# labhamlet/wavjepa

Measured on AMD Instinct MI355X. Metric: jepa_pretrain_clips_per_sec, higher is better.
Workload: dtype bf16

## Files before the change

### include/wavjepa_hip.h

```cpp
#ifndef WAVJEPA_HIP_H
#define WAVJEPA_HIP_H
#include <stdint.h>

#ifdef __cplusplus
extern "C" {
#endif

#define WJ_ABI_VERSION 16
int wj_abi_version(void);
int wj_device_count(void);
int wj_struct_size(const char* name);

enum {
    WJ_EPI_BF16 = 0,
    WJ_EPI_BIAS_GELU2 = 1,
    WJ_EPI_MUL_GELU_GRAD = 2,
    WJ_EPI_ADD_F32 = 3,
    WJ_EPI_ATOMIC_F32 = 4,
    WJ_EPI_CONV_GELU = 5,
    WJ_EPI_BIAS_GELU = 6,
    WJ_EPI_BF16_ADD_POS = 8,
    WJ_EPI_MUL_GELU_GRAD_Z = 7
};
typedef struct {
    const void* A;
    const void* B;
    void* C;
    void* C2;
    const void* bias;
    const void* aux;
    float* colsum;
    const int32_t* rowmap;
    int64_t lda, ldb, ldc;
    int32_t M, N, K;
    int32_t a_trans, b_trans;
    int32_t epilogue;
    int32_t split_k;
    int32_t seg_rows, seg_valid;
    float alpha;
    void* workspace;
    int64_t workspace_bytes;
    int32_t schedule;
    int32_t persist_cus;
} wj_gemm_args;
int wj_gemm_bf16(const wj_gemm_args*, void* stream);
int wj_gemm_release_stream(void* stream);
typedef struct {
    const void* A;
    const void* B;
    const void* scale_a;
    const void* scale_b;
    void* C;
    void* C2;
    const float* bias;
    void* q_out;
    void* q_scales;
    int64_t lda, ldb, ldc;
    int64_t ld_scale_a, ld_scale_b, ld_q_scale;
    int32_t M, N, K;
    int32_t epilogue;
} wj_gemm_fp8_args;
int wj_gemm_mxfp8(const wj_gemm_fp8_args*, void* stream);

typedef struct {
    const void* x;
    void* q;
    void* scales;
    int64_t ldx, ldq, ld_scale;
    int32_t M, K;
} wj_quantize_fp8_args;
int wj_quantize_mxfp8(const wj_quantize_fp8_args*, void* stream);

typedef struct {
    const void* A[8];
    const void* B[8];
    void* C[8];
    int64_t lda[8], ldb[8], ldc[8];
    int32_t M[8], N[8], K[8];
    int32_t n;
} wj_wgrad_group_args;
int wj_wgrad_grouped(const wj_wgrad_group_args*, void* stream);

// ... 379 lines not shown
```

### wavjepa_amd/csrc/gemm_panel.hip

```cpp
#include <atomic>
#include "common.h"
#include "../../include/wavjepa_hip.h"
#include "gemm_internal.h"

namespace {

constexpr int NT = 512;
constexpr int PN = 384;
constexpr int THIRDS = PN / 128;
constexpr unsigned SLOT = 16384u;
constexpr unsigned A_RING = 0u, B_RING = 4u * SLOT;
constexpr unsigned BIAS_OFF = 8u * SLOT;
constexpr unsigned STRIP_OFF = BIAS_OFF + 2048u;
constexpr unsigned STRIP_ROW = 144u;
constexpr int LDS_TOTAL = (int)(STRIP_OFF + 8u * 16u * STRIP_ROW);
constexpr int EPI_STORES = 4 * THIRDS;

typedef __attribute__((ext_vector_type(4))) unsigned u32x4;
typedef __attribute__((ext_vector_type(2))) unsigned u32x2;

struct QArgs {
    const char* A;
    const char* B;
    char* C;
    const float* bias;
    long ldc_b;
    unsigned lda_b, ldb_b;
    int M, K, nitems, wpx;
    int diag;
};

template <int N>
__device__ __forceinline__ void wait_vmcnt() {
    asm volatile("s_waitcnt vmcnt(%0)" ::"n"(N) : "memory");
}

__device__ __forceinline__ void dma(unsigned voff, const char* sbase, unsigned lds_dst) {
    asm volatile("s_mov_b32 m0, %2\n\ts_nop 0\n\tglobal_load_lds_dwordx4 %0, %1" ::"v"(voff), "s"(sbase), "s"(lds_dst) : "memory", "m0");
}

__device__ __forceinline__ unsigned pack_bf16(float a, float b) {
    bf16x2 p;
    p[0] = f2bf(a);
    p[1] = f2bf(b);
    return __builtin_bit_cast(unsigned, p);
}

struct Cursor {
    int b_kt, b_sub;
    int a_it, a_kt;
};

template <int SUB, int PB, int PA>
__device__ __forceinline__ void step(f32x4 (&acc)[4][2 * THIRDS], bf16x8 (&af)[2][4][2], bf16x8 (&bf)[2][2][2], char* smem, const QArgs& a,
                                     Cursor& cur, unsigned& slot_b, unsigned& slot_a, int nk, int n_my, int q0, int cstart,
                                     const unsigned (&voff)[4], const unsigned (&dpiece)[4], unsigned a_rd, unsigned b_rd, bool a_wave,
                                     int& lag_w, int& lag_a, int rot) {
    __builtin_amdgcn_sched_barrier(0);
    if (!a_wave) {
        if (lag_w > 0) { wait_vmcnt<8 + EPI_STORES>(); --lag_w; }
        else wait_vmcnt<8>();
    } else if constexpr (SUB == THIRDS - 1) {
        if (lag_a > 0) { wait_vmcnt<12 + EPI_STORES>(); --lag_a; }
        else wait_vmcnt<12>();
    }
    asm volatile("s_waitcnt lgkmcnt(0)" ::: "memory");
    __builtin_amdgcn_s_barrier();
    __builtin_amdgcn_sched_barrier(0);
    {
        const int bk = cur.b_kt + rot < nk ? cur.b_kt + rot : cur.b_kt + rot - nk;
        const char* sb = a.B + (long)(cur.b_sub * 128) * a.ldb_b + (long)bk * 128;
        const unsigned dst = B_RING + slot_b * SLOT;
        if (!a_wave) {
            const char* src = (WJ_LAB_BUILD && (a.diag & 1)) ? a.B : sb;
            const unsigned mask = (WJ_LAB_BUILD && (a.diag & 1)) ? 0u : ~0u;
#pragma unroll
            for (int u = 0; u < 4; ++u) dma(voff[u] & mask, src, dpiece[u] + dst);
        }
        slot_b = (slot_b + 1) & 3;
        if (++cur.b_sub == THIRDS) { cur.b_sub = 0; if (++cur.b_kt == nk) cur.b_kt = 0; }
    }
    if constexpr (SUB == 0) {
        const int it = cur.a_it < n_my ? cur.a_it : n_my - 1;
        const int m0 = min((cstart + q0 + it * a.wpx) * 128, a.M - 128);
        const int ak = cur.a_kt + rot < nk ? cur.a_kt + rot : cur.a_kt + rot - nk;
        const char* sa = a.A + (long)m0 * a.lda_b + (long)ak * 128;
        const unsigned dst = A_RING + slot_a * SLOT;
        if (a_wave) {
            const char* src = (WJ_LAB_BUILD && (a.diag & 2)) ? a.A : sa;
            const unsigned mask = (WJ_LAB_BUILD && (a.diag & 2)) ? 0u : ~0u;
#pragma unroll
            for (int u = 0; u < 4; ++u) dma(voff[u] & mask, src, dpiece[u] + dst);
        }
        slot_a = (slot_a + 1) & 3;
        if (++cur.a_kt == nk) { cur.a_kt = 0; ++cur.a_it; }
    }
// ... 28 lines not shown
    __builtin_amdgcn_sched_barrier(0);
}

__device__ __forceinline__ void epilogue(f32x4 (&acc)[4][2 * THIRDS], char* smem, const QArgs& a, int m0, int wave, int lane) {
    const int wm = wave >> 2, wn = wave & 3;
    const int i = lane & 15, g = lane >> 4;
    char* strip = smem + STRIP_OFF + wave * (16 * STRIP_ROW);
    char* wr = strip + i * STRIP_ROW + g * 8;
    const int srow = lane >> 2, schunk = lane & 3;
    const char* rd = strip + srow * STRIP_ROW + schunk * 16;
    char* c0 = a.C + (long)(m0 + wm * 64 + srow) * a.ldc_b + (long)(wn * 32) * 2 + schunk * 16;
    const float* bias = reinterpret_cast<const float*>(smem + BIAS_OFF) + wn * 32 + 4 * g;
#pragma unroll
    for (int t = 0; t < THIRDS; ++t) {
        f32x4 bv[2];
#pragma unroll
        for (int ni = 0; ni < 2; ++ni) bv[ni] = *reinterpret_cast<const f32x4*>(bias + t * 128 + ni * 16);
#pragma unroll
        for (int mi = 0; mi < 4; ++mi) {
#pragma unroll
            for (int ni = 0; ni < 2; ++ni) {
                const f32x4 v = acc[mi][t * 2 + ni] + bv[ni];
                *reinterpret_cast<u32x2*>(wr + ni * 32) = u32x2{pack_bf16(v[0], v[1]), pack_bf16(v[2], v[3])};
            }
            __builtin_amdgcn_wave_barrier();
            const u32x4 o = *reinterpret_cast<const u32x4*>(rd);
            __builtin_amdgcn_wave_barrier();
            char* dst = (WJ_LAB_BUILD && (a.diag & 16)) ? a.C + (lane & 7) * 16 : c0 + (long)(mi * 16) * a.ldc_b + (long)(t * 128) * 2;
            __builtin_nontemporal_store(o, reinterpret_cast<u32x4*>(dst));
        }
    }
}

__global__ __launch_bounds__(NT, 1) void gemm_panel_kernel(QArgs a) {
    extern __shared__ __attribute__((aligned(16))) char smem[];
    const int t = threadIdx.x, lane = t & 63;
    const int wave = __builtin_amdgcn_readfirstlane(t >> 6);
    const int wm = wave >> 2, wn = wave & 3;
    const bool a_wave = wave < 4;
    const int nk = a.K >> 6;
    const unsigned lds0 = (unsigned)(size_t)(__attribute__((address_space(3))) char*)smem;

    const int xl = blockIdx.x & 7, q0 = blockIdx.x >> 3;
    const int qn = a.nitems >> 3, qr = a.nitems & 7;
    const int clen = qn + (xl < qr ? 1 : 0);
    const int cstart = xl < qr ? xl * (qn + 1) : qr * (qn + 1) + (xl - qr) * qn;
    if (q0 >= clen) return;
    const int n_my = (clen - q0 + a.wpx - 1) / a.wpx;

    if (t < PN) reinterpret_cast<float*>(smem + BIAS_OFF)[t] = a.bias ? a.bias[t] : 0.f;

    unsigned dpiece[4], voff[4];
    const unsigned ld_b = a_wave ? a.lda_b : a.ldb_b;
#pragma unroll
    for (int u = 0; u < 4; ++u) {
        const int r0 = 32 * (wave & 3) + 8 * u;
        dpiece[u] = lds0 + (unsigned)r0 * 128u;
        const int row = r0 + (lane >> 3);
        voff[u] = (unsigned)row * ld_b + (unsigned)(((lane & 7) ^ ((row >> 1) & 7)) * 16);
    }
    const int i = lane & 15, g = lane >> 4;
    const unsigned sw = (unsigned)((g ^ ((i >> 1) & 7)) << 4);
    const unsigned a_rd = (unsigned)((wm * 64 + i) * 128) + sw;
    const unsigned b_rd = (unsigned)((wn * 32 + i) * 128) + sw;

    const int rot = (WJ_LAB_BUILD && (a.diag & 32)) ? (q0 + 3 * xl) % nk : 0;
    auto phys = [&](int kt) { return kt + rot < nk ? kt + rot : kt + rot - nk; };
    Cursor cur;
    cur.a_it = 0; cur.a_kt = 4; cur.b_kt = 1; cur.b_sub = 1;
    if (cur.a_kt == nk) { cur.a_kt = 0; cur.a_it = 1; }
    {
        const int m0 = min((cstart + q0) * 128, a.M - 128);
#pragma unroll
        for (int k = 0; k < 4; ++k) {
            if (a_wave) {
                const char* sa = a.A + (long)m0 * a.lda_b + (long)phys(k) * 128;
#pragma unroll
                for (int u = 0; u < 4; ++u) dma(voff[u], sa, dpiece[u] + A_RING + k * SLOT);
            } else {
                const int kt = k / THIRDS, sub = k - kt * THIRDS;
                const char* sb = a.B + (long)(sub * 128) * a.ldb_b + (long)phys(kt) * 128;
#pragma unroll
                for (int u = 0; u < 4; ++u) dma(voff[u], sb, dpiece[u] + B_RING + k * SLOT);
            }
        }
    }
    f32x4 acc[4][2 * THIRDS];
    bf16x8 af[2][4][2], bf[2][2][2];
    wait_vmcnt<12>();
    asm volatile("s_waitcnt lgkmcnt(0)" ::: "memory");
    __builtin_amdgcn_s_barrier();
    __builtin_amdgcn_sched_barrier(0);
#pragma unroll
    for (int ni = 0; ni < 2; ++ni) {
        bf[0][ni][0] = *reinterpret_cast<const bf16x8*>(smem + B_RING + b_rd + ni * 2048);
        bf[0][ni][1] = *reinterpret_cast<const bf16x8*>(smem + B_RING + (b_rd ^ 64u) + ni * 2048);
    }
#pragma unroll
    for (int mi = 0; mi < 4; ++mi) {
        af[0][mi][0] = *reinterpret_cast<const bf16x8*>(smem + A_RING + a_rd + mi * 2048);
        af[0][mi][1] = *reinterpret_cast<const bf16x8*>(smem + A_RING + (a_rd ^ 64u) + mi * 2048);
    }
    unsigned slot_b = 0, slot_a = 0;
    int lag_w = 0, lag_a = 0;

    for (int it = 0; it < n_my; ++it) {
        const int m0 = min((cstart + q0 + it * a.wpx) * 128, a.M - 128);
#pragma unroll
        for (int mi = 0; mi < 4; ++mi)
#pragma unroll
            for (int c = 0; c < 2 * THIRDS; ++c) acc[mi][c] = f32x4{0.f, 0.f, 0.f, 0.f};
        for (int kt = 0; kt < nk; kt += 2) {
            step<0, 0, 0>(acc, af, bf, smem, a, cur, slot_b, slot_a, nk, n_my, q0, cstart, voff, dpiece, a_rd, b_rd, a_wave, lag_w, lag_a, rot);
            step<1, 1, 0>(acc, af, bf, smem, a, cur, slot_b, slot_a, nk, n_my, q0, cstart, voff, dpiece, a_rd, b_rd, a_wave, lag_w, lag_a, rot);
            step<2, 0, 0>(acc, af, bf, smem, a, cur, slot_b, slot_a, nk, n_my, q0, cstart, voff, dpiece, a_rd, b_rd, a_wave, lag_w, lag_a, rot);
            step<0, 1, 1>(acc, af, bf, smem, a, cur, slot_b, slot_a, nk, n_my, q0, cstart, voff, dpiece, a_rd, b_rd, a_wave, lag_w, lag_a, rot);
            step<1, 0, 1>(acc, af, bf, smem, a, cur, slot_b, slot_a, nk, n_my, q0, cstart, voff, dpiece, a_rd, b_rd, a_wave, lag_w, lag_a, rot);
            step<2, 1, 1>(acc, af, bf, smem, a, cur, slot_b, slot_a, nk, n_my, q0, cstart, voff, dpiece, a_rd, b_rd, a_wave, lag_w, lag_a, rot);
        }
        __builtin_amdgcn_sched_barrier(0);
        asm volatile("s_nop 7\n\ts_nop 7" ::: "memory");
        epilogue(acc, smem, a, m0, wave, lane);
        __builtin_amdgcn_sched_barrier(0);
        lag_w = 3;
        lag_a = 3;
    }
    wait_vmcnt<0>();
    __builtin_amdgcn_s_barrier();
}


}

bool wj_gemm_panel_eligible(const wj_gemm_args* a) {
    if (a->a_trans || a->b_trans || a->rowmap || a->split_k > 1 || a->colsum || a->aux) return false;
    if (a->epilogue != WJ_EPI_BF16) return false;
    if (a->N != PN || a->M < 128) return false;
    if (a->K < 256 || (a->K % 128)) return false;
    if ((a->lda & 7) || (a->ldb & 7) || (a->ldc & 7)) return false;
    if (((uintptr_t)a->A | (uintptr_t)a->B | (uintptr_t)a->C | (uintptr_t)a->bias) & 15) return false;
    if (a->lda * 2 * 128 >= (1l << 31) || a->ldb * 2 * 128 >= (1l << 31)) return false;
    return true;
}

int wj_gemm_panel_launch(const wj_gemm_args* a, hipStream_t s) {
    if (!wj_gemm_panel_eligible(a)) return WJ_ERR_UNSUPPORTED;
    QArgs p;
    p.A = (const char*)a->A; p.B = (const char*)a->B; p.C = (char*)a->C; p.bias = (const float*)a->bias;
    p.ldc_b = a->ldc * 2; p.lda_b = (unsigned)(a->lda * 2); p.ldb_b = (unsigned)(a->ldb * 2);
    p.M = a->M; p.K = a->K;
    p.nitems = (a->M + 127) / 128;
    p.wpx = a->persist_cus > 0 ? (a->persist_cus > 32 ? 32 : a->persist_cus) : 32;
    p.diag = wj_lab_env_int("WJ_PANEL_DIAG", 0);
    int dev = 0;
    if (hipGetDevice(&dev) != hipSuccess || dev < 0 || dev >= 32) return WJ_ERR_UNSUPPORTED;
    static std::atomic<bool> lds_ok[32];
    if (!lds_ok[dev].load(std::memory_order_acquire)) {
        if (hipFuncSetAttribute((const void*)gemm_panel_kernel, hipFuncAttributeMaxDynamicSharedMemorySize, LDS_TOTAL) != hipSuccess) return WJ_ERR_LAUNCH;
        lds_ok[dev].store(true, std::memory_order_release);
    }
    hipLaunchKernelGGL(gemm_panel_kernel, dim3(8 * p.wpx), dim3(NT), LDS_TOTAL, s, p);
    WJ_CHECK_LAUNCH();
    return WJ_OK;
}
```

### wavjepa_amd/csrc/misc.hip

```cpp
#include <string.h>
#include "common.h"
#include "../../include/wavjepa_hip.h"
#ifdef WJ_LAB
#include "../../include/wavjepa_hip_lab.h"
#endif

namespace {

inline int grid_for(long n_items, int per_block, int cap = 8192) {
    long g = (n_items + per_block - 1) / per_block;
    if (g < 1) g = 1;
    return (int)(g > cap ? cap : g);
}

__global__ __launch_bounds__(256) void gelu_bwd_kernel(const bf16_t* __restrict__ dpost, const bf16_t* __restrict__ pre,
                                                       bf16_t* __restrict__ dpre, long n8) {
    for (long i = blockIdx.x * 256L + threadIdx.x; i < n8; i += (long)gridDim.x * 256) {
        const bf16x8 d = *reinterpret_cast<const bf16x8*>(dpost + i * 8);
        const bf16x8 p = *reinterpret_cast<const bf16x8*>(pre + i * 8);
        bf16x8 o;
#pragma unroll
        for (int e = 0; e < 8; ++e) o[e] = f2bf(bf2f(d[e]) * gelu_grad_f(bf2f(p[e])));
        *reinterpret_cast<bf16x8*>(dpre + i * 8) = o;
    }
// ... 506 lines not shown
        const int c = (int)(i / a.length), l = (int)(i - (long)c * a.length);
        const float d = src[(long)c * a.L_full + start + l] - mean;
        q += d * d;
    }
    const float stdv = sqrtf(block_sum(q, red) / (float)(n - 1));
    const float inv = 1.0f / (stdv + 1e-5f);
    const int orow = a.perm_inv ? a.perm_inv[bs] : bs;
    bf16_t* out = (bf16_t*)a.out + (long)orow * n;
    for (long i = threadIdx.x; i < n; i += 1024) {
        const int c = (int)(i / a.length), l = (int)(i - (long)c * a.length);
        out[i] = f2bf((src[(long)c * a.L_full + start + l] - mean) * inv);
    }
}

}

#define STREAM ((hipStream_t)stream)

extern "C" int wj_abi_version(void) { return WJ_ABI_VERSION; }
extern "C" int wj_device_count(void) {
    int n = 0;
    if (hipGetDeviceCount(&n) != hipSuccess) return 0;
    return n;
}

extern "C" int wj_struct_size(const char* name) {
    if (!name) return -1;
#define WJ_SZ(T) if (!strcmp(name, #T)) return (int)sizeof(T);
    WJ_SZ(wj_gemm_args) WJ_SZ(wj_ln_fwd_args) WJ_SZ(wj_ln_bwd_args) WJ_SZ(wj_colsum_args) WJ_SZ(wj_attn_fwd_args)
    WJ_SZ(wj_attn_bwd_args) WJ_SZ(wj_conv0_fwd_args) WJ_SZ(wj_conv0_bwd_args) WJ_SZ(wj_gelu_bwd_args) WJ_SZ(wj_conv_w_args)
    WJ_SZ(wj_add_pos_args) WJ_SZ(wj_gather_args) WJ_SZ(wj_scatter_fill_args) WJ_SZ(wj_scatter_fill_bwd_args)
    WJ_SZ(wj_unmask_rows_args) WJ_SZ(wj_instnorm_args) WJ_SZ(wj_mse_args) WJ_SZ(wj_ema_args) WJ_SZ(wj_sumsq_args)
    WJ_SZ(wj_adamw_args) WJ_SZ(wj_cast_args) WJ_SZ(wj_crop_args) WJ_SZ(wj_zero_rows_args) WJ_SZ(wj_instnorm_mean_args) WJ_SZ(wj_spin_args)
    WJ_SZ(wj_gemm_fp8_args) WJ_SZ(wj_quantize_fp8_args) WJ_SZ(wj_wgrad_group_args) WJ_SZ(wj_rir_conv_args) WJ_SZ(wj_snr_mix_args) WJ_SZ(wj_resample_args) WJ_SZ(wj_mse_groups_args) WJ_SZ(wj_transpose_args) WJ_SZ(wj_colsum_group_args) WJ_SZ(wj_rccl_init_args) WJ_SZ(wj_rccl_launch_args) WJ_SZ(wj_rccl_wait_args)
#ifdef WJ_LAB
    WJ_SZ(wj_collective_footprint_args)
#endif
#undef WJ_SZ
    return -1;
}

int64_t wj_gemm_ws_bytes(const wj_gemm_args* a);
int64_t wj_conv0_fwd_ws_bytes(const wj_conv0_fwd_args* a);
int64_t wj_conv0_bwd_ws_bytes(const wj_conv0_bwd_args* a);
int64_t wj_rir_conv_ws_bytes(const wj_rir_conv_args* a);
int64_t wj_snr_mix_ws_bytes(const wj_snr_mix_args* a);
int64_t wj_mse_groups_ws_bytes(const wj_mse_groups_args* a);

extern "C" int64_t wj_workspace_bytes(const char* fn, const void* args) {
    if (!fn || !args) return -1;
    if (!strcmp(fn, "wj_gemm_bf16")) return wj_gemm_ws_bytes((const wj_gemm_args*)args);
    if (!strcmp(fn, "wj_mask_scatter_fill_pos_bwd")) {
        const wj_scatter_fill_bwd_args* a = (const wj_scatter_fill_bwd_args*)args;
        return (int64_t)wj_scatter_fill_bwd_partial_rows(a->B, a->T) * a->D * 4;
    }
    if (!strcmp(fn, "wj_layernorm_bwd")) return 1536LL * 3 * ((const wj_ln_bwd_args*)args)->D * 4;
    if (!strcmp(fn, "wj_attn_bwd")) {
        const wj_attn_bwd_args* a = (const wj_attn_bwd_args*)args;
        return (int64_t)a->B * 3 * a->H * a->hd * 4;
    }
    if (!strcmp(fn, "wj_conv0_gn_gelu_fwd")) return wj_conv0_fwd_ws_bytes((const wj_conv0_fwd_args*)args);
    if (!strcmp(fn, "wj_conv0_gn_gelu_bwd")) return wj_conv0_bwd_ws_bytes((const wj_conv0_bwd_args*)args);
    if (!strcmp(fn, "wj_masked_mse")) {
        const wj_mse_args* a = (const wj_mse_args*)args;
        return (2 + (int64_t)a->B * a->G * a->T) * 4;
    }
    if (!strcmp(fn, "wj_grad_sumsq")) return 1024 * 4;
// ... 257 lines not shown
```

### wavjepa_amd/engine.py

```python
from __future__ import annotations

from dataclasses import dataclass
from typing import Dict, List, Optional, Sequence, Tuple

import numpy as np
import torch

from . import ops
from .params import FlatParams


def _empty(*shape, dtype, device):
    import os
    if os.environ.get("WJ_ARENA_FILL", "") == "nan":
        if not dtype.is_floating_point:
            return torch.full(shape, 0x7f, dtype=dtype, device=device)
        return torch.full(shape, float("nan"), dtype=dtype, device=device)
    return torch.empty(*shape, dtype=dtype, device=device)


@dataclass
class EngineConfig:
    conv_spec: Sequence[Tuple[int, int, int]]
    in_channels: int
# ... 249 lines not shown
        self.stacks = list(cfg.conv_prefixes)
        assert len(self.stacks) in (1, self.S)
        self.C = cfg.conv_spec[-1][0]
        assert all(c == self.C for c, _, _ in cfg.conv_spec), "all conv layers must have the same width"
        assert cfg.d_enc % cfg.h_enc == 0 and cfg.d_dec % cfg.h_dec == 0
        self.N = 0
        self.G = 0
        import os as _os
        self.use_side = _os.environ.get("WJ_SIDE_STREAM", "1") != "0"
        self._opt_ev = None
        self.ragged = _os.environ.get("WJ_RAGGED", "1") != "0"
        self.ragged_step = False
        self.sparse_conv = _os.environ.get("WJ_SPARSE_CONV", "1") != "0" and all(k >= st for _, k, st in cfg.conv_spec[1:])
        self._conv_grads_dirty = False
        self.fuse_conv_gelu_bwd = _os.environ.get("WJ_FUSE_CONV_GELU_BWD", "1") != "0"
        self.trim_tail = _os.environ.get("WJ_TRIM_TAIL", "1") != "0"
        self.tail = None
        self.fp8 = _os.environ.get("WJ_FP8", "0") == "1"
        self._w8: Dict[int, Tuple[torch.Tensor, torch.Tensor, int, int]] = {}
        self._a8: Dict[str, Tuple[torch.Tensor, torch.Tensor]] = {}
        self.side = self._pick_side_stream() if self.use_side else torch.cuda.Stream(device=self.dev)
        self.has_mapper = "post_extraction_mapper.weight" in flat.by_name
        self.wt_dgrad = _os.environ.get("WJ_WT_DGRAD", "1") != "0"
        self.pair_split = _os.environ.get("WJ_PAIR_SPLIT", "0") == "1"
        self.pair_ws = None
        self._conv_w_fresh = False
        self.defer_folds = _os.environ.get("WJ_DEFER_FOLDS", "1") != "0"
        self.fuse_add_pos = _os.environ.get("WJ_FUSE_ADD_POS", "1") != "0"
        self.mapper_wgrad_side = _os.environ.get("WJ_MAPPER_WGRAD_SIDE", "1") != "0"
        self.conv_wgrad_side = _os.environ.get("WJ_CONV_WGRAD_SIDE", "1") != "0"
        lean = _os.environ.get("WJ_LN_LEAN", "")
        self.ln_lean = {t.strip() for t in lean.replace("+", ",").split(",") if t.strip() and t.strip() != "0"} if self.use_side else set()
        self.ln_lean_wgs = int(_os.environ.get("WJ_LN_LEAN_WGS", "256"))
        self._lean_now = False
        self._folds = []
        self._bind_params()
        self._bind_wt()
        self._conv_w: Dict[str, torch.Tensor] = {}
        self._alloc_conv_weights()

    def _pick_side_stream(self) -> torch.cuda.Stream:
        main = torch.cuda.current_stream(self.dev)
        ticks = 20000
        ops.spin(100, stream=main.cuda_stream)

        def pair_ms(cand: torch.cuda.Stream) -> float:
            e0, e1, go, done = (torch.cuda.Event(enable_timing=True) for _ in range(4))
            best = 1e9
            for _ in range(2):
                go.record(main)
                cand.wait_event(go)
                e0.record(main)
                ops.spin(ticks, stream=main.cuda_stream)
                ops.spin(ticks, stream=cand.cuda_stream)
                done.record(cand)
                main.wait_event(done)
                e1.record(main)
                e1.synchronize()
                best = min(best, e0.elapsed_time(e1))
            return best

        def single_ms() -> float:
            e0, e1 = torch.cuda.Event(enable_timing=True), torch.cuda.Event(enable_timing=True)
            e0.record(main)
            ops.spin(ticks, stream=main.cuda_stream)
            e1.record(main)
# ... 271 lines not shown
        self.d_ctx_in = _empty(Me, c.d_enc, dtype=bf, device=dev)
        self.d_lf_b = _empty(M, c.d_enc, dtype=bf, device=dev)
        self.d_fn = _empty(M, C, dtype=f32, device=dev)

    def _layer_fwd(self, w: _Layer, a: _Acts, x_in: torch.Tensor, xb_in: torch.Tensor, M: int, D: int, H: int, B: int,
                   mask: Optional[torch.Tensor], seq: Optional[Tuple[torch.Tensor, int]] = None, save: bool = True,
                   x2_out: Optional[torch.Tensor] = None, x2_stats: Optional[torch.Tensor] = None,
                   sub: Optional[Tuple[torch.Tensor, torch.Tensor, int]] = None, stack: str = "enc", xq_ready: bool = False) -> bool:
        eps = self.cfg.ln_eps
        f8 = self.fp8 and w.wqkv in self._w8
        if not f8:
            xq_ready = False
            self._linear_fwd(stack, xb_in, w.wqkv, a.qkv, M=M, N=3 * D, K=D, bias=w.bqkv)
        else:
            qb, sb = self._a8[stack]
            qs, ss = self._a8s[stack]
            if not xq_ready:
                ops.quantize_mxfp8(xb_in, qs, ss, M=M, K=D, ldx=D, ldq=D, ld_scale=M)
            self._gemm8(qs, ss, w.wqkv, a.qkv, M=M, N=3 * D, K=D, bias=w.bqkv)
        if seq is not None:
            ops.attn_fwd(a.qkv, a.o, B=B, T=seq[1], H=H, hd=D // H, seq_off=seq[0], lse=a.lse if save else None)
        else:
            ops.attn_fwd(a.qkv, a.o, B=B, T=self.T, H=H, hd=D // H, key_mask=mask, lse=a.lse if save else None)
        o_in = a.o
        if sub is not None:
            rows, _, M = sub
            ops.mask_gather_rows(a.o, rows, self.tail_o, n_rows=M, D=D, elem_bytes=2)
            ops.mask_gather_rows(x_in, rows, self.tail_x, n_rows=M, D=D, elem_bytes=4)
            o_in, x_in = self.tail_o, self.tail_x
        f8_out = dict(y_fp8=qs, y_fp8_scales=ss, ld_fp8_scale=M) if f8 else {}
        if f8:
            ops.quantize_mxfp8(o_in, qs, ss, M=M, K=D, ldx=D, ldq=D, ld_scale=M)
            self._gemm8(qs, ss, w.wo, a.p, M=M, N=D, K=D, bias=w.bo)
        else:
            self._linear_fwd(stack, o_in, w.wo, a.p, M=M, N=D, K=D, bias=w.bo)
        lean = self.ln_lean_wgs if (self._lean_now and stack in self.ln_lean and not f8) else 0
        ops.layernorm_fwd(x_in, w.g1, w.be1, M=M, D=D, eps=eps, r=a.p, y_f32=a.x1, y_bf16=a.x1b, mean=a.m1, rstd=a.r1, workgroups=lean, **f8_out)
        if f8:
            gq = dict(q_out=qb, q_scales=sb, ld_q_scale=M)
            if save:
                self._gemm8(qs, ss, w.w1, a.h, M=M, N=4 * D, K=D, bias=w.b1, epilogue=ops.EPI_BIAS_GELU2, C2=a.g, **gq)
            else:
                self._gemm8(qs, ss, w.w1, None, M=M, N=4 * D, K=D, bias=w.b1, epilogue=ops.EPI_BIAS_GELU, **gq)
            self._gemm8(qb, sb, w.w2, a.f, M=M, N=D, K=4 * D, bias=w.b2)
        else:
            if save:
                self._linear_fwd(stack, a.x1b, w.w1, a.h, M=M, N=4 * D, K=D, bias=w.b1, epilogue=ops.EPI_BIAS_GELU2, C2=a.g)
            else:
                self._linear_fwd(stack, a.x1b, w.w1, a.g, M=M, N=4 * D, K=D, bias=w.b1, epilogue=ops.EPI_BIAS_GELU)
            self._linear_fwd(stack, a.g, w.w2, a.f, M=M, N=D, K=4 * D, bias=w.b2)
        ops.layernorm_fwd(a.x1, w.g2, w.be2, M=M, D=D, eps=eps, r=a.f, y_f32=a.x2 if x2_out is None else x2_out, y_bf16=a.x2b,
                          mean=a.m2, rstd=a.r2, group_stats=x2_stats, group_rows=self.T if x2_stats is not None else 0,
                          workgroups=lean if x2_stats is None else 0, **f8_out)
        return f8 and sub is None

    def _gemm8(self, q, sc, w_ptr: int, out, *, M: int, N: int, K: int, bias, epilogue: int = ops.EPI_BF16, C2=None, **extra) -> None:
        w8 = self._w8[w_ptr]
        ops.gemm_mxfp8(q, w8[0], sc, w8[1], out, M=M, N=N, K=K, lda=K, ldb=K, ldc=N, ld_scale_a=M, ld_scale_b=N, epilogue=epilogue, C2=C2,
                       bias=bias, **extra)

    def set_wt_need(self, rows_enc: int, rows_dec: int) -> None:
        self._wt_need = (self._wt_keys(rows_enc, self.cfg.d_enc, pairs=True), self._wt_keys(rows_dec, self.cfg.d_dec) if self.dec_layers else ())
        self._wt_live = {id(w): self._wt_need[0] for w in self.enc_layers}
        self._wt_live.update({id(w): self._wt_need[1] for w in self.dec_layers})

    def refresh_wt(self) -> None:
        need = self._wt_need
        if not self.wt_dgrad or self._wt_fresh == need:
            return
        if need not in self._wt_tables:
            f, rows, tiles = self.flat, [], 0
            for layers, keys in ((self.enc_layers, need[0]), (self.dec_layers, need[1])):
                for w in layers:
                    for k in keys:
                        sl = f.by_name[getattr(w, k + "_name")]
                        r, cc = sl.shape
                        rows.append((sl.offset, r, cc, tiles))
                        tiles += (r // 64) * (cc // 64)
            self._wt_tables[need] = (torch.tensor(rows, dtype=torch.int64, device=self.dev) if rows else None, len(rows), tiles)
        table, n_mats, n_tiles = self._wt_tables[need]
        if n_mats:
            ops.transpose_bf16(self.flat.p16, self.p16t, table, n_mats, n_tiles)
# ... 563 lines not shown
```

### wavjepa_amd/ops.py

```python
from __future__ import annotations

import ctypes
from typing import Optional, Union

import torch

from . import _abi
from ._abi import ENUMS, STRUCTS

Ptr = Union[torch.Tensor, int, None]

EPI_BF16 = ENUMS["WJ_EPI_BF16"]
EPI_BIAS_GELU2 = ENUMS["WJ_EPI_BIAS_GELU2"]
EPI_MUL_GELU_GRAD = ENUMS["WJ_EPI_MUL_GELU_GRAD"]
EPI_ADD_F32 = ENUMS["WJ_EPI_ADD_F32"]
EPI_ATOMIC_F32 = ENUMS["WJ_EPI_ATOMIC_F32"]
EPI_CONV_GELU = ENUMS["WJ_EPI_CONV_GELU"]
EPI_BIAS_GELU = ENUMS["WJ_EPI_BIAS_GELU"]
EPI_MUL_GELU_GRAD_Z = ENUMS["WJ_EPI_MUL_GELU_GRAD_Z"]
EPI_BF16_ADD_POS = ENUMS["WJ_EPI_BF16_ADD_POS"]
GROUP_STATS_SPLIT = _abi.DEFINES["WJ_GROUP_STATS_SPLIT"]
COLSUM_GROUP_MAX = _abi.DEFINES["WJ_COLSUM_GROUP_MAX"]


# ... 145 lines not shown


def transpose_bf16(src: Ptr, dst: Ptr, table: torch.Tensor, n_mats: int, n_tiles: int, stream: Optional[int] = None) -> None:
    _run("wj_transpose_bf16", "wj_transpose_args", stream, src=_p(src), dst=_p(dst), table=_p(table), n_mats=n_mats, n_tiles=n_tiles)


def gemm_set_persist_cus(workgroups_per_xcd: int) -> int:
    global _PERSIST_CUS
    import os
    prev = _PERSIST_CUS or max(1, min(32, int(os.environ.get("WJ_PERSIST_CUS", "32") or 32)))
    if workgroups_per_xcd > 0:
        _PERSIST_CUS = min(32, int(workgroups_per_xcd))
    return prev


def pick_split_k(M: int, N: int, K: int) -> int:
    bn = 256 if N % 256 == 0 else 128
    tiles = ((M + 255) // 256) * ((N + bn - 1) // bn)
    target = 256 if bn == 256 else 512
    s = max(1, (target + tiles // 2) // max(1, tiles))
    return max(1, min(s, (K + 1023) // 1024))


def layernorm_fwd(x: Ptr, gamma: Ptr, beta: Ptr, *, M: int, D: int, eps: float, r: Ptr = None, y_f32: Ptr = None,
                  y_bf16: Ptr = None, mean: Ptr = None, rstd: Ptr = None, x_is_bf16: bool = False, in_seg: int = 0,
                  in_valid: int = 0, group_stats: Ptr = None, group_rows: int = 0, in_chan: int = 0, y_fp8: Ptr = None,
                  y_fp8_scales: Ptr = None, ld_fp8_scale: int = 0, workgroups: int = 0, stream: Optional[int] = None) -> None:
    _run("wj_layernorm_fwd", "wj_ln_fwd_args", stream, x=_p(x), r=_p(r), gamma=_p(gamma), beta=_p(beta), y_f32=_p(y_f32),
         y_bf16=_p(y_bf16), mean=_p(mean), rstd=_p(rstd), group_stats=_p(group_stats), y_fp8=_p(y_fp8), y_fp8_scales=_p(y_fp8_scales),
         ld_fp8_scale=ld_fp8_scale, M=M, D=D, x_is_bf16=int(x_is_bf16), in_seg=in_seg, in_valid=in_valid, group_rows=group_rows,
         in_chan=in_chan, eps=eps, workgroups=int(workgroups))


def layernorm_bwd(dy: Ptr, x: Ptr, gamma: Ptr, mean: Ptr, rstd: Ptr, *, M: int, D: int, r: Ptr = None, dy2: Ptr = None,
                  ds_f32: Ptr = None, ds_bf16: Ptr = None, dgamma: Ptr = None, dbeta: Ptr = None, dbias: Ptr = None,
                  x_is_bf16: bool = False, in_seg: int = 0, in_valid: int = 0, out_seg: int = 0, out_valid: int = 0,
                  chan: int = 0, workspace: Ptr = None, dy2_is_bf16: bool = False, stream: Optional[int] = None) -> None:
    _run("wj_layernorm_bwd", "wj_ln_bwd_args", stream, dy=_p(dy), dy2=_p(dy2), dy2_is_bf16=int(dy2_is_bf16), x=_p(x), r=_p(r), gamma=_p(gamma),
         mean=_p(mean), rstd=_p(rstd), ds_f32=_p(ds_f32), ds_bf16=_p(ds_bf16), dgamma=_p(dgamma), dbeta=_p(dbeta),
         dbias=_p(dbias), workspace=_p(workspace), M=M, D=D, x_is_bf16=int(x_is_bf16), in_seg=in_seg, in_valid=in_valid, out_seg=out_seg,
         out_valid=out_valid, chan=chan)


def ln_bwd_partial_rows(M: int, D: int) -> int:
    return int(_abi.load().wj_ln_bwd_partial_rows(int(M), int(D)))


def colsum_f32_group(items, stream: Optional[int] = None) -> None:
    a = STRUCTS["wj_colsum_group_args"]()
    for i, (x, ldx, M, N, o0, o1, o2, n_each) in enumerate(items):
        a.x[i], a.o0[i], a.o1[i], a.o2[i] = _p(x), _p(o0), _p(o1), _p(o2)
        a.ldx[i], a.M[i], a.N[i], a.n_each[i] = ldx, M, N, n_each
    a.n = len(items)
    s = _stream() if stream is None else stream
    if PROFILE is None:
        _abi.call("wj_colsum_f32_group", a, s)
        return
    e0, e1 = TimingEvent(), TimingEvent()
    e0.record(s)
    _abi.call("wj_colsum_f32_group", a, s)
    e1.record(s)
    PROFILE.append(("wj_colsum_f32_group", dict(n=len(items)), e0, e1))


def rccl_unique_id() -> bytes:
    import ctypes
# ... 198 lines not shown
```

Baseline: 5639.

## Fuse decoder output-projection and FFN-down GEMMs with residual add and LayerNorm

Adds a LayerNorm-fused variant of the persistent panel GEMM (N=384). Its epilogue adds bias, writes the bf16 GEMM output, adds the residual and computes row mean and variance through a cross-wave LDS reduction. It then writes normalized fp32 and bf16 outputs plus the mean and rstd. The decoder stack uses it by default for the attention-output and FFN-down layers, removing separate layernorm kernel launches and the re-read of the GEMM output. In exchange the epilogue gets heavier, uses more LDS, and increases the vmcnt lag accounting in the main loop.

```diff
diff --git a/include/wavjepa_hip.h b/include/wavjepa_hip.h
--- a/include/wavjepa_hip.h
+++ b/include/wavjepa_hip.h
@@ -6,7 +6,7 @@
 extern "C" {
 #endif
 
-#define WJ_ABI_VERSION 16
+#define WJ_ABI_VERSION 17
 int wj_abi_version(void);
 int wj_device_count(void);
 int wj_struct_size(const char* name);
@@ -48,6 +48,24 @@
 typedef struct {
     const void* A;
     const void* B;
+    const float* bias;
+    void* r;
+    const float* x;
+    const float* gamma;
+    const float* beta;
+    float* y_f32;
+    void* y_bf16;
+    float* mean;
+    float* rstd;
+    int64_t lda, ldb;
+    int32_t M, N, K;
+    float eps;
+    int32_t persist_cus;
+} wj_gemm_ln_fwd_args;
+int wj_gemm_ln_fwd(const wj_gemm_ln_fwd_args*, void* stream);
+typedef struct {
+    const void* A;
+    const void* B;
     const void* scale_a;
     const void* scale_b;
     void* C;
diff --git a/wavjepa_amd/csrc/gemm_panel.hip b/wavjepa_amd/csrc/gemm_panel.hip
--- a/wavjepa_amd/csrc/gemm_panel.hip
+++ b/wavjepa_amd/csrc/gemm_panel.hip
@@ -15,6 +15,12 @@
 constexpr unsigned STRIP_ROW = 144u;
 constexpr int LDS_TOTAL = (int)(STRIP_OFF + 8u * 16u * STRIP_ROW);
 constexpr int EPI_STORES = 4 * THIRDS;
+constexpr unsigned GAMMA_OFF = (unsigned)LDS_TOTAL, BETA_OFF = GAMMA_OFF + 4u * PN;
+constexpr unsigned RED_OFF = BETA_OFF + 4u * PN;
+constexpr int LDS_TOTAL_LN = (int)(RED_OFF + 2u * 4u * 128u * 4u);
+constexpr int EPI_STORES_LN = 4 * THIRDS * 4 + 1;
+static_assert(LDS_TOTAL_LN <= 160 * 1024, "LDS");
+static_assert(12 + EPI_STORES_LN <= 63, "vmcnt field");
 
 typedef __attribute__((ext_vector_type(4))) unsigned u32x4;
 typedef __attribute__((ext_vector_type(2))) unsigned u32x2;
@@ -27,6 +33,14 @@
     long ldc_b;
     unsigned lda_b, ldb_b;
     int M, K, nitems, wpx;
+    const float* x;
+    const float* gamma;
+    const float* beta;
+    float* y32;
+    char* yb;
+    float* mean;
+    float* rstd;
+    float eps;
     int diag;
 };
 
@@ -51,17 +65,17 @@
     int a_it, a_kt;
 };
 
-template <int SUB, int PB, int PA>
+template <int SUB, int PB, int PA, int ES>
 __device__ __forceinline__ void step(f32x4 (&acc)[4][2 * THIRDS], bf16x8 (&af)[2][4][2], bf16x8 (&bf)[2][2][2], char* smem, const QArgs& a,
                                      Cursor& cur, unsigned& slot_b, unsigned& slot_a, int nk, int n_my, int q0, int cstart,
                                      const unsigned (&voff)[4], const unsigned (&dpiece)[4], unsigned a_rd, unsigned b_rd, bool a_wave,
                                      int& lag_w, int& lag_a, int rot) {
     __builtin_amdgcn_sched_barrier(0);
     if (!a_wave) {
-        if (lag_w > 0) { wait_vmcnt<8 + EPI_STORES>(); --lag_w; }
+        if (lag_w > 0) { wait_vmcnt<8 + ES>(); --lag_w; }
         else wait_vmcnt<8>();
     } else if constexpr (SUB == THIRDS - 1) {
-        if (lag_a > 0) { wait_vmcnt<12 + EPI_STORES>(); --lag_a; }
+        if (lag_a > 0) { wait_vmcnt<12 + ES>(); --lag_a; }
         else wait_vmcnt<12>();
     }
     asm volatile("s_waitcnt lgkmcnt(0)" ::: "memory");
@@ -156,7 +170,140 @@
     }
 }
 
+__device__ __forceinline__ void strip_store(unsigned w00, unsigned w01, unsigned w10, unsigned w11, char* wr, const char* rd, char* dst,
+                                            bool nt) {
+    *reinterpret_cast<u32x2*>(wr) = u32x2{w00, w01};
+    *reinterpret_cast<u32x2*>(wr + 32) = u32x2{w10, w11};
+    __builtin_amdgcn_wave_barrier();
+    const u32x4 o = *reinterpret_cast<const u32x4*>(rd);
+    __builtin_amdgcn_wave_barrier();
+    if (nt) __builtin_nontemporal_store(o, reinterpret_cast<u32x4*>(dst));
+    else *reinterpret_cast<u32x4*>(dst) = o;
+}
+
+__device__ __forceinline__ void row_sums(float (&v)[4], float* red, int wm, int wn, int i, int g) {
+#pragma unroll
+    for (int mi = 0; mi < 4; ++mi) {
+        v[mi] += __shfl_xor(v[mi], 16, 64);
+        v[mi] += __shfl_xor(v[mi], 32, 64);
+    }
+    if (g == 0) {
+#pragma unroll
+        for (int mi = 0; mi < 4; ++mi) red[wn * 128 + wm * 64 + mi * 16 + i] = v[mi];
+    }
+    asm volatile("s_waitcnt lgkmcnt(0)" ::: "memory");
+    __builtin_amdgcn_s_barrier();
+    asm volatile("" ::: "memory");
+#pragma unroll
+    for (int mi = 0; mi < 4; ++mi) {
+        const int row = wm * 64 + mi * 16 + i;
+        v[mi] = ((red[row] + red[128 + row]) + red[256 + row]) + red[384 + row];
+    }
+}
+
+__device__ __forceinline__ void epilogue_ln(f32x4 (&acc)[4][2 * THIRDS], char* smem, const QArgs& a, int m0, int wave, int lane) {
+    const int wm = wave >> 2, wn = wave & 3;
+    const int i = lane & 15, g = lane >> 4;
+    char* strip = smem + STRIP_OFF + wave * (16 * STRIP_ROW);
+    char* wr = strip + i * STRIP_ROW + g * 8;
+    const int srow = lane >> 2, schunk = lane & 3;
+    const char* rd = strip + srow * STRIP_ROW + schunk * 16;
+    const long so = (long)(m0 + wm * 64 + srow) * a.ldc_b + (long)(wn * 32) * 2 + schunk * 16;
+    const long eo = (long)(m0 + wm * 64 + i) * PN + wn * 32 + 4 * g;
+    const int cb = wn * 32 + 4 * g;
+    const float* bias = reinterpret_cast<const float*>(smem + BIAS_OFF) + cb;
+    const float* gam = reinterpret_cast<const float*>(smem + GAMMA_OFF) + cb;
+    const float* bet = reinterpret_cast<const float*>(smem + BETA_OFF) + cb;
+    float* red = reinterpret_cast<float*>(smem + RED_OFF);
+    constexpr float invD = 1.0f / (float)PN;
+
+    float rs[4] = {0.f, 0.f, 0.f, 0.f};
+    f32x4 xv[2][4][2];
+#pragma unroll
+    for (int mi = 0; mi < 4; ++mi)
+#pragma unroll
+        for (int ni = 0; ni < 2; ++ni) xv[0][mi][ni] = *reinterpret_cast<const f32x4*>(a.x + eo + (long)(mi * 16) * PN + ni * 16);
+#pragma unroll
+    for (int t = 0; t < THIRDS; ++t) {
+        if (t + 1 < THIRDS) {
+#pragma unroll
+            for (int mi = 0; mi < 4; ++mi)
+#pragma unroll
+                for (int ni = 0; ni < 2; ++ni)
+                    xv[(t + 1) & 1][mi][ni] = *reinterpret_cast<const f32x4*>(a.x + eo + (long)(mi * 16) * PN + (t + 1) * 128 + ni * 16);
+        }
+        f32x4 bv[2];
+#pragma unroll
+        for (int ni = 0; ni < 2; ++ni) bv[ni] = *reinterpret_cast<const f32x4*>(bias + t * 128 + ni * 16);
+#pragma unroll
+        for (int mi = 0; mi < 4; ++mi) {
+            unsigned w[2][2];
+#pragma unroll
+            for (int ni = 0; ni < 2; ++ni) {
+                const f32x4 h = acc[mi][t * 2 + ni] + bv[ni];
+                bf16x4 hb;
+#pragma unroll
+                for (int e = 0; e < 4; ++e) hb[e] = f2bf(h[e]);
+                f32x4 sv;
+#pragma unroll
+                for (int e = 0; e < 4; ++e) sv[e] = xv[t & 1][mi][ni][e] + bf2f(hb[e]);
+                rs[mi] += (sv[0] + sv[1]) + (sv[2] + sv[3]);
+                acc[mi][t * 2 + ni] = sv;
+                w[ni][0] = __builtin_bit_cast(unsigned, bf16x2{hb[0], hb[1]});
+                w[ni][1] = __builtin_bit_cast(unsigned, bf16x2{hb[2], hb[3]});
+            }
+            strip_store(w[0][0], w[0][1], w[1][0], w[1][1], wr, rd, a.C + so + (long)(mi * 16) * a.ldc_b + t * 256, true);
+        }
+    }
+    row_sums(rs, red, wm, wn, i, g);
+    float mean[4], rstd[4], sq[4];
+#pragma unroll
+    for (int mi = 0; mi < 4; ++mi) {
+        mean[mi] = rs[mi] * invD;
+        sq[mi] = 0.f;
+#pragma unroll
+        for (int c = 0; c < 2 * THIRDS; ++c)
+#pragma unroll
+            for (int e = 0; e < 4; ++e) {
+                const float d = acc[mi][c][e] - mean[mi];
+                sq[mi] += d * d;
+            }
+    }
+    row_sums(sq, red + 512, wm, wn, i, g);
+#pragma unroll
+    for (int mi = 0; mi < 4; ++mi) rstd[mi] = rsqrtf(sq[mi] * invD + a.eps);
+#pragma unroll
+    for (int t = 0; t < THIRDS; ++t) {
+        f32x4 gv[2], bt[2];
+#pragma unroll
+        for (int ni = 0; ni < 2; ++ni) {
+            gv[ni] = *reinterpret_cast<const f32x4*>(gam + t * 128 + ni * 16);
+            bt[ni] = *reinterpret_cast<const f32x4*>(bet + t * 128 + ni * 16);
+        }
+#pragma unroll
+        for (int mi = 0; mi < 4; ++mi) {
+            unsigned w[2][2];
+#pragma unroll
+            for (int ni = 0; ni < 2; ++ni) {
+                f32x4 y;
+#pragma unroll
+                for (int e = 0; e < 4; ++e) y[e] = (acc[mi][t * 2 + ni][e] - mean[mi]) * rstd[mi] * gv[ni][e] + bt[ni][e];
+                __builtin_nontemporal_store(y, reinterpret_cast<f32x4*>(a.y32 + eo + (long)(mi * 16) * PN + t * 128 + ni * 16));
+                w[ni][0] = pack_bf16(y[0], y[1]);
+                w[ni][1] = pack_bf16(y[2], y[3]);
+            }
+            strip_store(w[0][0], w[0][1], w[1][0], w[1][1], wr, rd, a.yb + so + (long)(mi * 16) * a.ldc_b + t * 256, false);
+        }
+    }
+    const bool st_rstd = (wn & 1) != 0;
+    const float mv = g == 0 ? mean[0] : (g == 1 ? mean[1] : (g == 2 ? mean[2] : mean[3]));
+    const float rv = g == 0 ? rstd[0] : (g == 1 ? rstd[1] : (g == 2 ? rstd[2] : rstd[3]));
+    (st_rstd ? a.rstd : a.mean)[m0 + wm * 64 + g * 16 + i] = st_rstd ? rv : mv;
+}
+
+template <bool LN>
 __global__ __launch_bounds__(NT, 1) void gemm_panel_kernel(QArgs a) {
+    constexpr int ES = LN ? EPI_STORES_LN : EPI_STORES;
     extern __shared__ __attribute__((aligned(16))) char smem[];
     const int t = threadIdx.x, lane = t & 63;
     const int wave = __builtin_amdgcn_readfirstlane(t >> 6);
@@ -173,6 +320,10 @@
     const int n_my = (clen - q0 + a.wpx - 1) / a.wpx;
 
     if (t < PN) reinterpret_cast<float*>(smem + BIAS_OFF)[t] = a.bias ? a.bias[t] : 0.f;
+    if (LN && t < PN) {
+        reinterpret_cast<float*>(smem + GAMMA_OFF)[t] = a.gamma[t];
+        reinterpret_cast<float*>(smem + BETA_OFF)[t] = a.beta[t];
+    }
 
     unsigned dpiece[4], voff[4];
     const unsigned ld_b = a_wave ? a.lda_b : a.ldb_b;
@@ -235,16 +386,17 @@
 #pragma unroll
             for (int c = 0; c < 2 * THIRDS; ++c) acc[mi][c] = f32x4{0.f, 0.f, 0.f, 0.f};
         for (int kt = 0; kt < nk; kt += 2) {
-            step<0, 0, 0>(acc, af, bf, smem, a, cur, slot_b, slot_a, nk, n_my, q0, cstart, voff, dpiece, a_rd, b_rd, a_wave, lag_w, lag_a, rot);
-            step<1, 1, 0>(acc, af, bf, smem, a, cur, slot_b, slot_a, nk, n_my, q0, cstart, voff, dpiece, a_rd, b_rd, a_wave, lag_w, lag_a, rot);
-            step<2, 0, 0>(acc, af, bf, smem, a, cur, slot_b, slot_a, nk, n_my, q0, cstart, voff, dpiece, a_rd, b_rd, a_wave, lag_w, lag_a, rot);
-            step<0, 1, 1>(acc, af, bf, smem, a, cur, slot_b, slot_a, nk, n_my, q0, cstart, voff, dpiece, a_rd, b_rd, a_wave, lag_w, lag_a, rot);
-            step<1, 0, 1>(acc, af, bf, smem, a, cur, slot_b, slot_a, nk, n_my, q0, cstart, voff, dpiece, a_rd, b_rd, a_wave, lag_w, lag_a, rot);
-            step<2, 1, 1>(acc, af, bf, smem, a, cur, slot_b, slot_a, nk, n_my, q0, cstart, voff, dpiece, a_rd, b_rd, a_wave, lag_w, lag_a, rot);
+            step<0, 0, 0, ES>(acc, af, bf, smem, a, cur, slot_b, slot_a, nk, n_my, q0, cstart, voff, dpiece, a_rd, b_rd, a_wave, lag_w, lag_a, rot);
+            step<1, 1, 0, ES>(acc, af, bf, smem, a, cur, slot_b, slot_a, nk, n_my, q0, cstart, voff, dpiece, a_rd, b_rd, a_wave, lag_w, lag_a, rot);
+            step<2, 0, 0, ES>(acc, af, bf, smem, a, cur, slot_b, slot_a, nk, n_my, q0, cstart, voff, dpiece, a_rd, b_rd, a_wave, lag_w, lag_a, rot);
+            step<0, 1, 1, ES>(acc, af, bf, smem, a, cur, slot_b, slot_a, nk, n_my, q0, cstart, voff, dpiece, a_rd, b_rd, a_wave, lag_w, lag_a, rot);
+            step<1, 0, 1, ES>(acc, af, bf, smem, a, cur, slot_b, slot_a, nk, n_my, q0, cstart, voff, dpiece, a_rd, b_rd, a_wave, lag_w, lag_a, rot);
+            step<2, 1, 1, ES>(acc, af, bf, smem, a, cur, slot_b, slot_a, nk, n_my, q0, cstart, voff, dpiece, a_rd, b_rd, a_wave, lag_w, lag_a, rot);
         }
         __builtin_amdgcn_sched_barrier(0);
         asm volatile("s_nop 7\n\ts_nop 7" ::: "memory");
-        epilogue(acc, smem, a, m0, wave, lane);
+        if constexpr (LN) epilogue_ln(acc, smem, a, m0, wave, lane);
+        else epilogue(acc, smem, a, m0, wave, lane);
         __builtin_amdgcn_sched_barrier(0);
         lag_w = 3;
         lag_a = 3;
@@ -267,23 +419,59 @@
     return true;
 }
 
+namespace {
+
+template <bool LN>
+int launch_panel(const QArgs& p, hipStream_t s) {
+    constexpr int lds = LN ? LDS_TOTAL_LN : LDS_TOTAL;
+    int dev = 0;
+    if (hipGetDevice(&dev) != hipSuccess || dev < 0 || dev >= 32) return WJ_ERR_UNSUPPORTED;
+    static std::atomic<bool> lds_ok[32];
+    if (!lds_ok[dev].load(std::memory_order_acquire)) {
+        if (hipFuncSetAttribute((const void*)gemm_panel_kernel<LN>, hipFuncAttributeMaxDynamicSharedMemorySize, lds) != hipSuccess) return WJ_ERR_LAUNCH;
+        lds_ok[dev].store(true, std::memory_order_release);
+    }
+    hipLaunchKernelGGL(gemm_panel_kernel<LN>, dim3(8 * p.wpx), dim3(NT), lds, s, p);
+    WJ_CHECK_LAUNCH();
+    return WJ_OK;
+}
+
+}
+
 int wj_gemm_panel_launch(const wj_gemm_args* a, hipStream_t s) {
     if (!wj_gemm_panel_eligible(a)) return WJ_ERR_UNSUPPORTED;
-    QArgs p;
+    QArgs p{};
     p.A = (const char*)a->A; p.B = (const char*)a->B; p.C = (char*)a->C; p.bias = (const float*)a->bias;
     p.ldc_b = a->ldc * 2; p.lda_b = (unsigned)(a->lda * 2); p.ldb_b = (unsigned)(a->ldb * 2);
     p.M = a->M; p.K = a->K;
     p.nitems = (a->M + 127) / 128;
-    p.wpx = a->persist_cus > 0 ? (a->persist_cus > 32 ? 32 : a->persist_cus) : 32;
+    p.wpx = wj_gemm_persist_wpx(a);
     p.diag = wj_lab_env_int("WJ_PANEL_DIAG", 0);
-    int dev = 0;
-    if (hipGetDevice(&dev) != hipSuccess || dev < 0 || dev >= 32) return WJ_ERR_UNSUPPORTED;
-    static std::atomic<bool> lds_ok[32];
-    if (!lds_ok[dev].load(std::memory_order_acquire)) {
-        if (hipFuncSetAttribute((const void*)gemm_panel_kernel, hipFuncAttributeMaxDynamicSharedMemorySize, LDS_TOTAL) != hipSuccess) return WJ_ERR_LAUNCH;
-        lds_ok[dev].store(true, std::memory_order_release);
-    }
-    hipLaunchKernelGGL(gemm_panel_kernel, dim3(8 * p.wpx), dim3(NT), LDS_TOTAL, s, p);
-    WJ_CHECK_LAUNCH();
-    return WJ_OK;
-}
+    return launch_panel<false>(p, s);
+}
+
+extern "C" int wj_gemm_ln_fwd(const wj_gemm_ln_fwd_args* a, void* stream) {
+    WJ_CLEAR_STALE_ERROR();
+    if (!a || !a->A || !a->B || !a->r || !a->x || !a->gamma || !a->beta || !a->y_f32 || !a->y_bf16 || !a->mean || !a->rstd) return WJ_ERR_ARG;
+    if (a->N != PN || a->M < 128 || a->K < 256 || (a->K % 128)) return WJ_ERR_ARG;
+    if (a->lda < a->K || a->ldb < a->K || (a->lda & 7) || (a->ldb & 7)) return WJ_ERR_ARG;
+    if (a->lda * 2 * 128 >= (1l << 31) || a->ldb * 2 * 128 >= (1l << 31)) return WJ_ERR_ARG;
+    if (((uintptr_t)a->A | (uintptr_t)a->B | (uintptr_t)a->bias | (uintptr_t)a->r | (uintptr_t)a->x | (uintptr_t)a->gamma |
+         (uintptr_t)a->beta | (uintptr_t)a->y_f32 | (uintptr_t)a->y_bf16) & 15)
+        return WJ_ERR_ARG;
+    if (((uintptr_t)a->mean | (uintptr_t)a->rstd) & 3) return WJ_ERR_ARG;
+    if ((const void*)a->x == a->r || (const void*)a->x == (const void*)a->y_f32 || (const void*)a->x == a->y_bf16) return WJ_ERR_ARG;
+    if (!(a->eps >= 0.f) || a->persist_cus < 0 || a->persist_cus > 32) return WJ_ERR_ARG;
+    wj_gemm_args g{};
+    g.persist_cus = a->persist_cus;
+    QArgs p{};
+    p.A = (const char*)a->A; p.B = (const char*)a->B; p.C = (char*)a->r; p.bias = a->bias;
+    p.ldc_b = PN * 2; p.lda_b = (unsigned)(a->lda * 2); p.ldb_b = (unsigned)(a->ldb * 2);
+    p.M = a->M; p.K = a->K;
+    p.nitems = (a->M + 127) / 128;
+    p.wpx = wj_gemm_persist_wpx(&g);
+    p.x = a->x; p.gamma = a->gamma; p.beta = a->beta;
+    p.y32 = a->y_f32; p.yb = (char*)a->y_bf16; p.mean = a->mean; p.rstd = a->rstd; p.eps = a->eps;
+    p.diag = 0;
+    return launch_panel<true>(p, (hipStream_t)stream);
+}
diff --git a/wavjepa_amd/csrc/misc.hip b/wavjepa_amd/csrc/misc.hip
--- a/wavjepa_amd/csrc/misc.hip
+++ b/wavjepa_amd/csrc/misc.hip
@@ -562,7 +562,7 @@
     WJ_SZ(wj_add_pos_args) WJ_SZ(wj_gather_args) WJ_SZ(wj_scatter_fill_args) WJ_SZ(wj_scatter_fill_bwd_args)
     WJ_SZ(wj_unmask_rows_args) WJ_SZ(wj_instnorm_args) WJ_SZ(wj_mse_args) WJ_SZ(wj_ema_args) WJ_SZ(wj_sumsq_args)
     WJ_SZ(wj_adamw_args) WJ_SZ(wj_cast_args) WJ_SZ(wj_crop_args) WJ_SZ(wj_zero_rows_args) WJ_SZ(wj_instnorm_mean_args) WJ_SZ(wj_spin_args)
-    WJ_SZ(wj_gemm_fp8_args) WJ_SZ(wj_quantize_fp8_args) WJ_SZ(wj_wgrad_group_args) WJ_SZ(wj_rir_conv_args) WJ_SZ(wj_snr_mix_args) WJ_SZ(wj_resample_args) WJ_SZ(wj_mse_groups_args) WJ_SZ(wj_transpose_args) WJ_SZ(wj_colsum_group_args) WJ_SZ(wj_rccl_init_args) WJ_SZ(wj_rccl_launch_args) WJ_SZ(wj_rccl_wait_args)
+    WJ_SZ(wj_gemm_fp8_args) WJ_SZ(wj_quantize_fp8_args) WJ_SZ(wj_wgrad_group_args) WJ_SZ(wj_rir_conv_args) WJ_SZ(wj_snr_mix_args) WJ_SZ(wj_resample_args) WJ_SZ(wj_mse_groups_args) WJ_SZ(wj_transpose_args) WJ_SZ(wj_colsum_group_args) WJ_SZ(wj_rccl_init_args) WJ_SZ(wj_rccl_launch_args) WJ_SZ(wj_rccl_wait_args) WJ_SZ(wj_gemm_ln_fwd_args)
 #ifdef WJ_LAB
     WJ_SZ(wj_collective_footprint_args)
 #endif
diff --git a/wavjepa_amd/engine.py b/wavjepa_amd/engine.py
--- a/wavjepa_amd/engine.py
+++ b/wavjepa_amd/engine.py
@@ -305,6 +305,7 @@
         lean = _os.environ.get("WJ_LN_LEAN", "")
         self.ln_lean = {t.strip() for t in lean.replace("+", ",").split(",") if t.strip() and t.strip() != "0"} if self.use_side else set()
         self.ln_lean_wgs = int(_os.environ.get("WJ_LN_LEAN_WGS", "256"))
+        self.fuse_gemm_ln = _os.environ.get("WJ_FUSE_GEMM_LN", "1") != "0"
         self._lean_now = False
         self._folds = []
         self._bind_params()
@@ -642,10 +643,15 @@
         if f8:
             ops.quantize_mxfp8(o_in, qs, ss, M=M, K=D, ldx=D, ldq=D, ld_scale=M)
             self._gemm8(qs, ss, w.wo, a.p, M=M, N=D, K=D, bias=w.bo)
-        else:
-            self._linear_fwd(stack, o_in, w.wo, a.p, M=M, N=D, K=D, bias=w.bo)
         lean = self.ln_lean_wgs if (self._lean_now and stack in self.ln_lean and not f8) else 0
-        ops.layernorm_fwd(x_in, w.g1, w.be1, M=M, D=D, eps=eps, r=a.p, y_f32=a.x1, y_bf16=a.x1b, mean=a.m1, rstd=a.r1, workgroups=lean, **f8_out)
+        fuse = self.fuse_gemm_ln and stack == "dec" and D == 384 and not f8 and not lean and M >= 128
+        if fuse:
+            ops.gemm_ln_fwd(o_in, w.wo, a.p, x_in, w.g1, w.be1, a.x1, a.x1b, a.m1, a.r1, M=M, K=D, eps=eps, bias=w.bo)
+        else:
+            if not f8:
+                self._linear_fwd(stack, o_in, w.wo, a.p, M=M, N=D, K=D, bias=w.bo)
+            ops.layernorm_fwd(x_in, w.g1, w.be1, M=M, D=D, eps=eps, r=a.p, y_f32=a.x1, y_bf16=a.x1b, mean=a.m1, rstd=a.r1, workgroups=lean,
+                              **f8_out)
         if f8:
             gq = dict(q_out=qb, q_scales=sb, ld_q_scale=M)
             if save:
@@ -658,6 +664,9 @@
                 self._linear_fwd(stack, a.x1b, w.w1, a.h, M=M, N=4 * D, K=D, bias=w.b1, epilogue=ops.EPI_BIAS_GELU2, C2=a.g)
             else:
                 self._linear_fwd(stack, a.x1b, w.w1, a.g, M=M, N=4 * D, K=D, bias=w.b1, epilogue=ops.EPI_BIAS_GELU)
+            if fuse and x2_out is None and x2_stats is None:
+                ops.gemm_ln_fwd(a.g, w.w2, a.f, a.x1, w.g2, w.be2, a.x2, a.x2b, a.m2, a.r2, M=M, K=4 * D, eps=eps, bias=w.b2)
+                return False
             self._linear_fwd(stack, a.g, w.w2, a.f, M=M, N=D, K=4 * D, bias=w.b2)
         ops.layernorm_fwd(a.x1, w.g2, w.be2, M=M, D=D, eps=eps, r=a.f, y_f32=a.x2 if x2_out is None else x2_out, y_bf16=a.x2b,
                           mean=a.m2, rstd=a.r2, group_stats=x2_stats, group_rows=self.T if x2_stats is not None else 0,
diff --git a/wavjepa_amd/ops.py b/wavjepa_amd/ops.py
--- a/wavjepa_amd/ops.py
+++ b/wavjepa_amd/ops.py
@@ -201,6 +201,14 @@
          in_chan=in_chan, eps=eps, workgroups=int(workgroups))
 
 
+
+def gemm_ln_fwd(A: Ptr, B: Ptr, r: Ptr, x: Ptr, gamma: Ptr, beta: Ptr, y_f32: Ptr, y_bf16: Ptr, mean: Ptr, rstd: Ptr, *, M: int,
+                K: int, eps: float, bias: Ptr = None, lda: Optional[int] = None, ldb: Optional[int] = None, N: int = 384,
+                persist_cus: Optional[int] = None, stream: Optional[int] = None) -> None:
+    _run("wj_gemm_ln_fwd", "wj_gemm_ln_fwd_args", stream, A=_p(A), B=_p(B), bias=_p(bias), r=_p(r), x=_p(x), gamma=_p(gamma),
+         beta=_p(beta), y_f32=_p(y_f32), y_bf16=_p(y_bf16), mean=_p(mean), rstd=_p(rstd), lda=K if lda is None else lda,
+         ldb=K if ldb is None else ldb, M=M, N=N, K=K, eps=eps, persist_cus=_PERSIST_CUS if persist_cus is None else int(persist_cus))
+
 def layernorm_bwd(dy: Ptr, x: Ptr, gamma: Ptr, mean: Ptr, rstd: Ptr, *, M: int, D: int, r: Ptr = None, dy2: Ptr = None,
                   ds_f32: Ptr = None, ds_bf16: Ptr = None, dgamma: Ptr = None, dbeta: Ptr = None, dbias: Ptr = None,
                   x_is_bf16: bool = False, in_seg: int = 0, in_valid: int = 0, out_seg: int = 0, out_valid: int = 0,
```

Result: no change. 5677 (median of 6 runs) (+0.7%).
